# SuperScientificSoftwareLaboratory/DASP

Measured on AMD Instinct MI355X. Metric: SpMV GFLOP/s (f64), higher is better.
Workload: dtype f64; 1 GPU; HV15R synthetic stand-in (seeded; SuiteSparse dims/row statistics), A=1, x=1; rows=2017169, cols=2017169, nnz=275454726, partition=single GPU, generator_rev=26e32ff958e7, y_candidates=1

## Files before the change

dasp_amd/_lib.py:

```python
import ctypes as C
import os
import subprocess

_HERE = os.path.dirname(os.path.abspath(__file__))
SO_PATH = os.environ.get("DASP_AMD_SO") or os.path.join(_HERE, "libdasp_amd.so")


class DaspError(RuntimeError):
    def __init__(self, status, msg):
        super().__init__("dasp status %d: %s" % (status, msg))
        self.status = status


class Options(C.Structure):
    _fields_ = [
        ("threshold", C.c_double), ("block_longest", C.c_int), ("y_order", C.c_int), ("long_piece", C.c_int),
        ("host_threads", C.c_int), ("n_parts", C.c_int), ("part_bounds", C.POINTER(C.c_int)), ("part_stride", C.c_int),
        ("x_window", C.c_int), ("row_window", C.c_int), ("cid16", C.c_int), ("stream_policy", C.c_int),
        ("col_panels", C.c_int), ("slab_max_len", C.c_int), ("x_window_hybrid", C.c_int), ("piece_min_len", C.c_int),
        ("chunk_pairs", C.c_int), ("cid8", C.c_int), ("short_seg", C.c_int), ("row_tile_max", C.c_int), ("sort_columns", C.c_int),
        ("two_phase", C.c_int), ("tp_col_block", C.c_int), ("tp_row_block", C.c_int), ("long_cb", C.c_int),
        ("value_map", C.c_int),
    ]

# ... 109 lines not shown
    L.dasp_plan_panel.restype = vp
    L.dasp_plan_panel_range.argtypes = [vp, C.c_int, ip, ip]
    L.dasp_plan_upload.argtypes = [vp]
    L.dasp_plan_drop_host.argtypes = [vp]
    L.dasp_plan_update_values.argtypes = [vp, vp, vp]
    L.dasp_plan_update_values_host.argtypes = [vp, vp]
    L.dasp_plan_value_map_slots.argtypes = [vp]
    L.dasp_plan_value_map_slots.restype = C.c_longlong
    if hasattr(L, "dasp_plan_csr_fetch_bytes"):
        L.dasp_plan_csr_fetch_bytes.argtypes = [vp]
        L.dasp_plan_csr_fetch_bytes.restype = C.c_longlong
    if hasattr(L, "dasp_plan_shared_ids"):
        L.dasp_plan_shared_ids.argtypes = [vp, C.POINTER(C.c_longlong), C.POINTER(C.c_longlong), ip]
        L.dasp_plan_shared_ids_export.argtypes = [vp, C.c_char_p, vp, C.c_size_t]
        L.dasp_plan_shared_ids_export.restype = C.c_longlong
    L.dasp_plan_set_stream_policy.argtypes = [vp, C.c_int]
    if hasattr(L, "dasp_plan_set_tp_exact"):
        L.dasp_plan_set_tp_exact.argtypes = [vp, C.c_int]
        L.dasp_plan_tp_exact.argtypes = [vp]
        L.dasp_tp_exact_dot_f16.argtypes = [vp, vp, C.c_longlong, C.c_int, C.c_uint16, C.POINTER(C.c_uint16)]
    if hasattr(L, "dasp_plan_set_hub_exact"):
        L.dasp_plan_set_hub_exact.argtypes = [vp, C.c_int]
        L.dasp_plan_hub_exact.argtypes = [vp]
    if hasattr(L, "dasp_plan_set_f32_vectors"):
        fp = C.POINTER(C.c_float)
        L.dasp_plan_set_f32_vectors.argtypes = [vp, C.c_int]
        L.dasp_plan_f32_vectors.argtypes = [vp]
        L.dasp_plan_spmv_f32.argtypes = [vp, fp, fp, vp]
        L.dasp_plan_spmv_acc_f32.argtypes = [vp, fp, fp, vp]
    if hasattr(L, "dasp_plan_spmv_semiring_f32"):
# ... 46 lines not shown
    L.dasp_synth_generator.restype = C.c_char_p
    L.dasp_synth_row_lengths.argtypes = [C.c_char_p, C.c_double, C.c_int, C.c_int, vp]
    L.dasp_synth_rows.argtypes = [C.c_char_p, C.c_double, C.c_int, C.c_int, vp, vp]
    _lib = L
    return L


def check(rc):
    if rc != 0:
        raise DaspError(rc, lib().dasp_last_error().decode("utf-8", "replace"))


EXPORTS = (
    "dasp_last_error dasp_version dasp_mmio_allinone_f64 dasp_mmio_allinone_f16 dasp_free dasp_csr_save dasp_csr_load dasp_options_default "
    "dasp_plan_create dasp_plan_create_device dasp_plan_download_array dasp_plan_destroy dasp_plan_save dasp_plan_load dasp_plan_order dasp_plan_stats dasp_plan_y_order dasp_plan_x_len dasp_plan_panel_count dasp_plan_panel dasp_plan_panel_range dasp_plan_host_array dasp_plan_upload dasp_plan_tune_placement "
    "dasp_plan_drop_host dasp_plan_update_values dasp_plan_update_values_host dasp_plan_value_map_slots dasp_plan_csr_fetch_bytes dasp_plan_shared_ids dasp_plan_shared_ids_export dasp_plan_set_stream_policy dasp_plan_set_tp_exact dasp_plan_tp_exact dasp_plan_set_hub_exact dasp_plan_hub_exact dasp_tp_exact_dot_f16 dasp_plan_spmv dasp_plan_spmv_acc dasp_plan_set_f32_vectors dasp_plan_f32_vectors dasp_plan_spmv_f32 dasp_plan_spmv_acc_f32 dasp_plan_spmv_semiring_f32 dasp_plan_time dasp_plan_time_each dasp_plan_time_graph dasp_spmv_all_f64 dasp_spmv_all_f16 dasp_partition_rows "
    "dasp_selftest_mfma dasp_synth_dims dasp_synth_generator dasp_synth_row_lengths dasp_synth_rows "
    "dasp_mg_unique_id dasp_mg_plan_create dasp_mg_destroy dasp_mg_upload dasp_mg_comm_init dasp_mg_set_x dasp_mg_spmv dasp_mg_product dasp_mg_allgather "
    "dasp_mg_wait dasp_mg_get_y dasp_mg_get_y_local dasp_mg_y_local dasp_mg_gathered dasp_mg_x dasp_mg_subplan dasp_mg_info dasp_mg_check dasp_mg_set_fused dasp_mg_set_fake_exchange "
    "dasp_mg_push_export dasp_mg_push_connect dasp_mg_set_exchange dasp_mg_push_loopback dasp_mg_reserved_stream").split()
```

dasp_amd/api.py:

```python
import ctypes as C
import os

import numpy as np

from . import _lib
from ._lib import DaspError, Options, Stats

Y_PERMUTED, Y_NATURAL = 0, 1
MIN_PLUS, MIN_SECOND = 1, 2


def _vp(a):
    return a.ctypes.data_as(C.c_void_p)


def _dtype(precision):
    if precision == 64:
        return np.float64
    if precision == 16:
        return np.float16
    raise ValueError("precision must be 64 or 16")


def mmio_allinone(filename, precision=64):
# ... 212 lines not shown
        return {"available": bool(rc), "paired_id_bytes": int(pb.value), "shared_bytes": int(sb.value), "in_use": bool(use.value)}

    def shared_ids_export(self):
        out = []
        for what in (b"plane", b"table"):
            n = int(_lib.lib().dasp_plan_shared_ids_export(self._h, what, None, 0))
            if n < 0:
                _lib.check(n)
            a = np.empty(n // 4, np.uint32)
            n2 = int(_lib.lib().dasp_plan_shared_ids_export(self._h, what, a.ctypes.data_as(C.c_void_p), a.nbytes))
            if n2 < 0:
                _lib.check(n2)
            out.append(a)
        return out[0], out[1].reshape(-1, 4)

    @property
    def value_map_slots(self):
        n = int(_lib.lib().dasp_plan_value_map_slots(self._h))
        if n < 0:
            _lib.check(n)
        return n

    def kernel_variant(self):
        name = _lib.lib().dasp_debug_plan_kernel(self._h)
        if name is None:
            raise _lib.DaspError(-22, _lib.lib().dasp_last_error().decode("utf-8", "replace"))
        return name.decode()

    def set_stream_policy(self, policy):
        _lib.check(_lib.lib().dasp_plan_set_stream_policy(self._h, int(policy)))
# ... 139 lines not shown
```

dasp_amd/csrc/capi.cpp:

```cpp
#include <hip/hip_runtime_api.h>

#include <algorithm>
#include <cstdio>
#include <cstdlib>
#include <cstring>
#include <exception>
#include <memory>
#include <new>
#include <string>
#include <sys/stat.h>
#include <vector>

#include "plan.hpp"
#include "device.hpp"
#include "tp_exact.hpp"

namespace dasp {
const char *last_error_cstr();
int upload_plan(Plan &p);
int tune_placement(Plan &p, int trials, const void *dX, void *dY, double *ms_first, double *ms_kept);
int launch_spmv(Plan &p, const void *dX, void *dY, void *stream, bool accumulate);
int time_spmv_each(Plan &p, const void *dX, void *dY, void *stream, int warmup, int iters, float *ms_each);
int time_spmv(Plan &p, const void *dX, void *dY, void *stream, int warmup, int iters, double *wall_ms, double *event_ms);
int time_spmv_graph(Plan &p, const void *dX, void *dY, void *stream, int warmup, int iters, int batch, double *wall_ms, double *event_ms);
// ... 292 lines not shown
    return guarded("dasp_plan_shared_ids", [&] {
        long long pb = 0, sb = 0;
        if (!p.sh_known) {
            SharedIds sh;
            (void)derive_shared_ids(p, sh);
            p.sh_paired_bytes = sh.paired_id_bytes; p.sh_shared_bytes = sh.shared_bytes; p.sh_known = true;
        }
        pb = p.sh_paired_bytes; sb = p.sh_shared_bytes;
        if (pb == 0) return 0;
        if (paired_id_bytes) *paired_id_bytes = pb;
        if (shared_bytes) *shared_bytes = sb;
        return 1;
    });
}

long long dasp_plan_shared_ids_export(const dasp_plan_t *plan, const char *what, void *dst, size_t bytes)
{
    if (!plan || !what) return DASP_ERR_ARG;
    long long need = 0;
    const int rc = guarded("dasp_plan_shared_ids_export", [&] {
        const bool plane = std::strcmp(what, "plane") == 0;
        if (!plane && std::strcmp(what, "table") != 0) { set_error("dasp_plan_shared_ids_export: \"plane\" or \"table\""); return (int)DASP_ERR_ARG; }
        SharedIds sh;
        if (!derive_shared_ids(plan->impl, sh)) { set_error("the plan has no shared id plane (f64 with 16-bit ids, host arrays present, at least one pipelined block)"); return (int)DASP_ERR_STATE; }
        const std::vector<uint32_t> &v = plane ? sh.plane : sh.table;
        need = (long long)v.size() * 4;
        if (dst && bytes >= (size_t)need && need > 0) std::memcpy(dst, v.data(), (size_t)need);
        return (int)DASP_OK;
    });
    return rc != DASP_OK ? (long long)rc : need;
}

int dasp_plan_upload(dasp_plan_t *plan)
{
    if (!plan) return DASP_ERR_ARG;
// ... 254 lines not shown
```

dasp_amd/csrc/device.hpp:

```cpp
#pragma once

#include <cstddef>
#include <vector>

#include "plan.hpp"

namespace dasp {

struct ShortDev {
    int len, count, tiles, tile0;
    long long elem_off;
    SlotMap map;
    int seg, rpt;
};

struct DevArgs {
    const void *x;
    void *y;
    const void *long_val; const int *long_cid; const int *piece_ptr; const int *piece_dst; void *partial;
    const int *multi_ptr; const int *multi_dst;
    int n_pieces, n_multi;
    int pair_mode;
    const int *med_ptr; const void *med_val; const int *med_cid;
    const unsigned short *med_cid16; const int *med_base;
// ... 14 lines not shown
    int short_tpw, n_short_waves;
    int grp_wave0[kNumShortGroups];
    int grp_tile0[kNumShortGroups];
    const int *order;
    int wg_long, wg_med, wg_short;
    int xcd_on;
    int xcd_blk[9];
    int med_stride;
    const void *rt_val; const int *rt_cid; const int *rt_ptr; const unsigned short *rt_start; const unsigned long long *rt_mask;
    int n_rt_tiles, wg_rt, rt_max;
    const unsigned short *long_cid16; const int *long_base; const int *piece_c16;
    const int *med_nt;
    int wg_rot;
    int win_tiles;
    const unsigned char *med_shplane; const unsigned *med_shtab;
};

struct TpDev {
    const unsigned short *lcol; const int *dst; const int *unit;
    const void *val; const unsigned short *lrow; void *xs;
    const int *rb_row0; const int *rb_seg0;
    int n_units, n_rb, cb, rb_max, xlen, m;
};

struct LcbDev {
    const void *val; const unsigned short *lcol; const int *ptr; const int *unit; const int *row_dst; void *partial;
    int n_units, n_rows, n_cb, cb, xlen;
    void *xpart;
    int xsteps;
};
// ... 7 lines not shown
    void *dargs = nullptr;
    void *args_sent = nullptr;
    void *arena = nullptr;
    size_t arena_bytes = 0;
    ArenaMap map{};
    DevArgs args{};
    TpDev tp{};
    LcbDev lcb{};
    void *lcb_xpart = nullptr;
    void *wide_xs = nullptr, *wide_part = nullptr;
    bool nt = false;
    bool win1 = false;
    bool seven_waves = false;
    bool long16 = false;
    bool shared_ids = false;
    int device = -1;
    size_t ypart_stride = 0;
    void *vm_map = nullptr, *vm_runs = nullptr;
    bool vm_ready = false;
    void *pk_map[7] = {};
    int vm_n_runs = 0;
    long long vm_blocks = 0, vm_slots = 0;
    std::vector<Plan *> vm_arenas;
};
int value_map_upload(Plan &p);
void value_map_free(DevicePlan *d);


int require_device();
int upload_plan(Plan &p);
// ... 48 lines not shown
```

dasp_amd/csrc/mgstep.hip:

```cpp
#include <hip/hip_runtime.h>

#include <algorithm>
#include <cstdlib>
#include <string>
#include <vector>

#include "spmv_device.hpp"
#include "mgx_device.hpp"

namespace dasp {

struct StepCtl {
    const unsigned long long *gathered;
    unsigned long long need;
    const unsigned char *mark;
    const unsigned *mark_members;
    int n_marked, n_mark_shards;
    unsigned *mark_shards, *mark_top;
    unsigned long long *own_go;
    unsigned *all_shards, *all_top;
    unsigned long long *ready;
    unsigned long long step;
    int *err;
    int grid_a, grid_b, n_poll;
// ... 177 lines not shown
        hipError_t e_ = (expr);                                                                \
        if (e_ != hipSuccess) {                                                                \
            set_error(std::string(#expr) + ": " + hipGetErrorString(e_));                      \
            return e_ == hipErrorNoDevice ? DASP_ERR_NO_DEVICE : DASP_ERR_HIP;                 \
        }                                                                                      \
    } while (0)

int launch_mg_step(Plan &own, Plan *other, const void *x_own, const void *x_gathered, void *y, const MgStepCtl &h, void *stream)
{
    if (!mg_step_supported(own, other)) { set_error("plans do not qualify for the fused multi-GPU step"); return DASP_ERR_STATE; }
    DevArgs a = own.dev->args, b = other ? other->dev->args : own.dev->args;
    a.x = x_own; a.y = y; a.acc = 0;
    b.x = x_gathered; b.y = y; b.acc = 0;
    a.wg_med = (a.n_blocks + kWavesPerWG - 1) / kWavesPerWG; a.xcd_on = 0;
    b.wg_med = (b.n_blocks + kWavesPerWG - 1) / kWavesPerWG; b.xcd_on = 0;
    StepCtl c{};
    char *w = static_cast<char *>(h.words);
    c.mark_shards = reinterpret_cast<unsigned *>(w); c.all_shards = reinterpret_cast<unsigned *>(w + 8192);
    c.mark_top = reinterpret_cast<unsigned *>(w + 16384); c.all_top = reinterpret_cast<unsigned *>(w + 16384 + 256);
    c.gathered = reinterpret_cast<const unsigned long long *>(w + kMgWordGathered); c.need = other ? h.need : 0;
    c.own_go = reinterpret_cast<unsigned long long *>(w + kMgWordOwnGo);
    c.ready = reinterpret_cast<unsigned long long *>(w + kMgWordReady); c.step = h.step; c.err = h.err ? static_cast<int *>(h.err) : reinterpret_cast<int *>(w + kMgWordErr);
    c.grid_a = a.wg_long + a.wg_med + a.wg_short;
    c.grid_b = other ? b.wg_long + b.wg_med + b.wg_short : 0;
    c.n_poll = std::min(c.grid_b, std::max(1, h.max_pollers));
    c.poll_at = std::max(0, std::min(c.grid_a, (int)((double)c.grid_a * h.poll_at)));
    c.xcd_fenced = reinterpret_cast<unsigned long long *>(w + kMgWordXcd);
    c.mark = static_cast<const unsigned char *>(h.mark); c.mark_members = static_cast<const unsigned *>(h.mark_members);
    c.n_marked = other ? h.n_marked : 0; c.n_mark_shards = h.n_mark_shards;
    c.blk_order = static_cast<const int *>(h.blk_order);
// ... 29 lines not shown
}

int launch_mg_flag(void *word, unsigned long long value, void *stream)
{
    hipLaunchKernelGGL(dasp_mg_flag_kernel, dim3(1), dim3(64), 0, static_cast<hipStream_t>(stream), static_cast<unsigned long long *>(word), value);
    HIP_TRY(hipGetLastError());
    return DASP_OK;
}

int launch_mg_step2(Plan &plan, const void *x, void *y, const MgStep2Ctl &h, const MgPushArgs &push, void *stream)
{
    if (!mg_step_supported(plan, nullptr)) { set_error("plan does not qualify for the one-stream multi-GPU step"); return DASP_ERR_STATE; }
    DevArgs a = plan.dev->args;
    a.x = x; a.y = y; a.acc = 0;
    a.wg_med = (a.n_blocks + kWavesPerWG - 1) / kWavesPerWG; a.xcd_on = 0;
    Step2Ctl c{};
    c.wg_list = static_cast<const int *>(h.wg_list); c.blk_order = static_cast<const int *>(h.blk_order);
    c.n_push = h.n_push; c.n_free = h.n_free; c.n_marked = h.n_marked; c.n_total = h.n_total;
    c.n_poll = h.max_pollers > 0 ? std::max(1, std::min(h.n_marked, h.max_pollers)) : 0;
    c.arrived = static_cast<const unsigned long long *>(h.arrived); c.world = h.world; c.rank = h.rank; c.need = h.need;
    c.err = static_cast<int *>(h.err); c.timeout = h.timeout_ticks; c.sleep = std::max(1, h.poll_sleep);
    c.fence_mode = h.fence_mode; c.xcd_fenced = static_cast<unsigned long long *>(h.xcd_fenced); c.step = h.step;
    if (c.n_total != a.wg_long + a.wg_med + a.wg_short || c.n_free + c.n_marked > c.n_total) { set_error("one-stream step: the workgroup list does not match the plan's grid"); return DASP_ERR_STATE; }
    if (c.n_poll == 0 && c.n_marked == 0 && c.need) c.n_poll = 1;
    const int grid = c.n_push + (c.n_poll ? c.n_total - c.n_marked + c.n_poll : c.n_total);
    hipStream_t s = static_cast<hipStream_t>(stream);
    if (plan.dev->nt) hipLaunchKernelGGL((dasp_mg_step2_kernel<true>), dim3(grid), dim3(256), 0, s, a, push, c);
    else hipLaunchKernelGGL((dasp_mg_step2_kernel<false>), dim3(grid), dim3(256), 0, s, a, push, c);
    HIP_TRY(hipGetLastError());
    return DASP_OK;
// ... 4 lines not shown
```

dasp_amd/csrc/plan.hpp:

```cpp
#pragma once

#include <cstddef>
#include <cstdint>
#include <memory>
#include <string>
#include <utility>
#include <vector>

#include "../../include/dasp_amd.h"

namespace dasp {

template <class T>
struct NoInit : std::allocator<T> {
    template <class U> struct rebind { using other = NoInit<U>; };
    NoInit() = default;
    template <class U> NoInit(const NoInit<U> &) {}
    template <class U> void construct(U *p) noexcept { ::new (static_cast<void *>(p)) U; }
    template <class U, class... A> void construct(U *p, A &&...a) { ::new (static_cast<void *>(p)) U(std::forward<A>(a)...); }
};
template <class T> using raw_vector = std::vector<T, NoInit<T>>;

constexpr int kWave = 64;
constexpr long long kStreamBytes = 256ll << 20;
// ... 221 lines not shown
    TwoPhase tp;
    bool tp_exact = false;
    bool hub_exact = false;
    bool f32_vectors = false;

    bool value_map = false;
    std::vector<uint32_t> long_map, med_map, irr_map, short_map, rt_map;
    const uint32_t *map_src = nullptr;
    bool loaded = false;

    bool host_dropped = false;
    long long csr_fetch_bytes = 0;
    mutable long long sh_paired_bytes = 0, sh_shared_bytes = 0;
    mutable bool sh_known = false;
    bool sh_in_use = false;
    DevicePlan *dev = nullptr;

    ~Plan();
};

struct SharedIds {
    std::vector<uint32_t> plane, table;
    long long paired_id_bytes = 0;
    long long shared_bytes = 0;
    int n_pipelined = 0;
};
bool shared_ids_qualify(const Plan &p);
bool derive_shared_ids(const Plan &p, SharedIds &out);

struct DevCsr { const int *rp, *ci; const void *val; const uint32_t *src = nullptr; };
struct PackMeta {
    const std::vector<int> *ridL = nullptr; const std::vector<long long> *startL = nullptr;
    const raw_vector<int> *ridM = nullptr, *lenM = nullptr;
    const std::vector<int> *glist[kNumShortGroups] = {};
};
int devpack_validate(const Plan &p, const DevCsr &d);
int devpack_window_spans(const Plan &p, const DevCsr &d, const raw_vector<int> &ridW, int R, int *lo, int *hi, long long *wnnz);
int devpack_line_scatter(const Plan &p, const DevCsr &d, const std::vector<int> &rows, long long *lines, long long *entries);
int devpack_row_coherence(const Plan &p, const DevCsr &d, const std::vector<int> &rows, int within, long long *near, long long *entries);
int devpack_chunk_spans(const Plan &p, const DevCsr &d, const raw_vector<int> &ridM, const raw_vector<int> &lenM,
                        const std::vector<int> &nchunks, int *k16, unsigned long long *narrow_mask);
int devpack_densest_spans(const Plan &p, const DevCsr &d, const raw_vector<int> &ridW, const raw_vector<int> &lenW, int R, const std::vector<int> &wlist,
                          long long cap_cols, int A, int *hmin, long long *hin);
// ... 72 lines not shown
```

dasp_amd/csrc/sharedids.cpp:

```cpp
#include <cstring>

#include "plan.hpp"

namespace dasp {

bool shared_ids_qualify(const Plan &p)
{
    if (p.precision != 64 || !p.cid16 || p.windowed || p.two_phase || !p.panels.empty() || p.panel || p.host_dropped) return false;
    const size_t nb = p.med_ptr.empty() ? 0 : p.med_ptr.size() - 1;
    if (nb == 0 || p.med_c8ptr.size() != nb + 1 || p.irr_ptr.size() < 2) return false;
    return p.med_cid8.size() == p.cnt_reg8 && p.med_cid16.size() == p.cnt_reg - p.cnt_reg8 && p.cnt_reg > 0;
}

bool derive_shared_ids(const Plan &p, SharedIds &out)
{
    out = SharedIds();
    if (!shared_ids_qualify(p)) return false;
    constexpr int CH = 64, K = 4;
    const size_t nb = p.med_ptr.size() - 1;
    out.table.assign(4 * nb, 0u);
    const unsigned char *c8 = p.med_cid8.data();
    const unsigned char *c16 = reinterpret_cast<const unsigned char *>(p.med_cid16.data());
    std::vector<const unsigned char *> slot;
    for (size_t b = 0; b < nb; ++b) {
// ... 27 lines not shown
        uint32_t *dst = out.plane.data() + at;
        for (const unsigned char *s : slot)
            for (int kq = 0; kq < 4; ++kq)
                for (int g = 0; g < L; ++g) std::memcpy(dst++, s + 4 * (rep[g] + 16 * kq), 4);
        out.table[4 * b] = (uint32_t)ranks; out.table[4 * b + 1] = (uint32_t)(ranks >> 32);
        out.table[4 * b + 2] = (uint32_t)(at / 4); out.table[4 * b + 3] = (uint32_t)L;
        out.paired_id_bytes += (long long)slot.size() * 4 * CH;
        ++out.n_pipelined;
        if (at / 4 > 0xFFFFFFFFull) { out = SharedIds(); return false; }
    }
    if (out.n_pipelined == 0) { out = SharedIds(); return false; }
    out.shared_bytes = (long long)out.plane.size() * 4 + (long long)out.table.size() * 4;
    return true;
}

}
```

dasp_amd/csrc/spmv_device.hpp:

```cpp
#pragma once
#include <hip/hip_runtime.h>

#include <cstdint>

#include "plan.hpp"
#include "device.hpp"

namespace dasp {

typedef double f64x4 __attribute__((ext_vector_type(4)));
typedef double f64x2 __attribute__((ext_vector_type(2)));
typedef float f32x4 __attribute__((ext_vector_type(4)));
typedef _Float16 f16x4 __attribute__((ext_vector_type(4)));
typedef int i32x4 __attribute__((ext_vector_type(4)));
typedef int i32x2 __attribute__((ext_vector_type(2)));
typedef unsigned short u16x4 __attribute__((ext_vector_type(4)));
typedef unsigned short u16x8 __attribute__((ext_vector_type(8)));
typedef const __attribute__((address_space(1))) unsigned char *gbyte_p;
typedef _Float16 f16x8 __attribute__((ext_vector_type(8)));


template <bool NT, class U>
__device__ __forceinline__ U ldg(const U *p)
{
// ... 56 lines not shown
template <class U> __device__ __forceinline__ U *ldp(U *const *field)
{
    typedef __attribute__((address_space(1))) U *gptr;
    return (U *)*reinterpret_cast<const __attribute__((address_space(4))) gptr *>(reinterpret_cast<uintptr_t>(field));
}
__device__ __forceinline__ DevArgs load_args(const CallArgs &c)
{
    static_assert(sizeof(DevArgs) % 4 == 0, "DevArgs is a whole number of words");
    int w[sizeof(DevArgs) / 4];
#pragma unroll
    for (int i = 0; i < (int)(sizeof(DevArgs) / 4); ++i) w[i] = tab<true>(reinterpret_cast<const int *>(c.plan), i);
    DevArgs a;
    __builtin_memcpy(&a, w, sizeof a);
#define DASP_G(f) a.f = ldp(&c.plan->f)
    DASP_G(long_val); DASP_G(long_cid); DASP_G(long_cid16); DASP_G(long_base); DASP_G(piece_c16); DASP_G(piece_ptr); DASP_G(piece_dst); DASP_G(partial); DASP_G(multi_ptr); DASP_G(multi_dst);
    DASP_G(med_ptr); DASP_G(med_val); DASP_G(med_cid); DASP_G(med_cid16); DASP_G(med_base); DASP_G(med_cid8); DASP_G(med_c8ptr); DASP_G(med_shplane); DASP_G(med_shtab);
    DASP_G(irr_ptr); DASP_G(med_nt); DASP_G(irr_val); DASP_G(irr_cid); DASP_G(med_dst); DASP_G(win_cmin); DASP_G(win_len);
    DASP_G(short_val); DASP_G(short_cid); DASP_G(groups); DASP_G(order);
    DASP_G(rt_val); DASP_G(rt_cid); DASP_G(rt_ptr); DASP_G(rt_start); DASP_G(rt_mask);
#undef DASP_G
    a.x = c.x; a.y = c.y; a.acc = c.acc; a.ywt = c.ywt;
    return a;
}

template <int I, int N> struct LastLE {
    static __device__ __forceinline__ void run(const int (&arr)[N], int w, int &idx, int &val)
    {
        if constexpr (I < N) { const bool in = w >= arr[I]; idx = in ? I : idx; val = in ? arr[I] : val; LastLE<I + 1, N>::run(arr, w, idx, val); }
    }
};
template <int I, int N> struct PickPair {
// ... 501 lines not shown
                for (int j = 0; j < 4; ++j) { f.a[j] = ok ? f.a[j] : (_Float16)0; f.b[j] = ok ? f.b[j] : (_Float16)0; }
            }
            frag_mfma(acc, f);
        }
    }
    part_t d;
    const bool on_diag = diag_of(acc, lane, d);
    const part_t total = wave_sum(on_diag ? d : (part_t)0);
    if (lane == 0) {
        const int dst = tab<true>(a.piece_dst, p);
        if (dst >= 0) put_y<T, YS>(a, dst, total);
        else static_cast<part_t *>(a.partial)[~dst] = total;
    }
}

template <class T, int L, bool NT, int YS = 0>
__device__ __forceinline__ void short_rows(const DevArgs &a, const ShortDev &g, int local_tile, int lane)
{
    constexpr int SR = Tr<T>::SHORT_ROWS;
    constexpr int V = SR / kWave;
    const T *x = static_cast<const T *>(a.x);
    const T *val = static_cast<const T *>(a.short_val);
    using part_t = typename Tr<T>::part_t;
    part_t s[V];
#pragma unroll
    for (int v = 0; v < V; ++v) s[v] = 0;
    const size_t base = (size_t)g.elem_off + (size_t)local_tile * L * SR + (size_t)V * lane;
#pragma unroll
    for (int k = 0; k < L; ++k) {
        if constexpr (V == 2) {
// ... 243 lines not shown
#ifndef DASP_WIN64_U
#define DASP_WIN64_U 3
#define DASP_WIN64_S 6
#endif
template <class T, bool NT, bool C16, bool WIN, bool C8, bool RT = false, bool W64 = false, bool L16 = false, bool SH = false>
__device__ __forceinline__ void spmv_body(const DevArgs &a, char *lds_raw, int wg_index, Stamps &st)
{
    const int lane = threadIdx.x & 63;
    const int wave = __builtin_amdgcn_readfirstlane(threadIdx.x >> 6);
    int wg = wg_index;
    if constexpr (sizeof(T) == 2 && !WIN && !RT) {
        if (a.wg_rot) { const int grid = a.wg_long + a.wg_med + a.wg_short; wg += a.wg_rot; wg = wg >= grid ? wg - grid : wg; }
    }
    const int wpw = WIN ? a.wpw : kWavesPerWG;
    if (wg < a.wg_long) {
        const int p = wg * wpw + wave;
        if (p < a.n_pieces) long_piece<T, NT, 0, !WIN, L16 && !WIN>(a, p, lane);
    } else if (wg < a.wg_long + a.wg_med) {
        st.kind = 1;
        if constexpr (!WIN) {
            const int m = wg - a.wg_long;
            const XGlobal<T> x{static_cast<const T *>(a.x)};
            if (a.xcd_on) {
                const int k = m & 7;
                int lo = a.xcd_blk[0], hi = a.xcd_blk[1];
                PickPair<1, 9>::run(a.xcd_blk, k, lo, hi);
                const int b = lo + (m >> 3) * kWavesPerWG + wave;
                if (b < hi) medium_block<T, NT, C16, 0, C8, 0, false, 0, 0, SH>(a, b, lane, x);
            } else if (sizeof(T) == 8 && !a.med_stride) {
                const int b = m * kWavesPerWG + wave;
                if (b < a.n_blocks) medium_block<T, NT, C16, 0, C8, 0, false, 0, 0, SH>(a, b, lane, x);
// ... 113 lines not shown
```

dasp_amd/csrc/upload.cpp:

```cpp
#include <hip/hip_runtime_api.h>

#include <algorithm>
#include <chrono>
#include <cmath>
#include <cstdio>
#include <cstdlib>
#include <cstring>
#include <string>
#include <type_traits>
#include <vector>

#include "plan.hpp"
#include "device.hpp"

namespace dasp {

#define HIP_TRY(expr)                                                                          \
    do {                                                                                       \
        hipError_t e_ = (expr);                                                                \
        if (e_ != hipSuccess) {                                                                \
            set_error(std::string(#expr) + ": " + hipGetErrorString(e_));                      \
            return e_ == hipErrorNoDevice ? DASP_ERR_NO_DEVICE : DASP_ERR_HIP;                 \
        }                                                                                      \
    } while (0)
// ... 82 lines not shown
    }
    if (narrow_elems) *narrow_elems = narrow;
    return on;
}
void choose_long16(Plan &p)
{
    DevicePlan *d = p.dev;
    if (!d) return;
    d->long16 = long16_rule(p, nullptr);
}

long long shared_ids_net_saving(const Plan &p, const SharedIds &s, bool long16)
{
    long long narrow = 0;
    (void)long16_rule(p, &narrow);
    return s.paired_id_bytes - s.shared_bytes - (long16 ? 2 * narrow : 0);
}
static bool seven_waves_rule(const Plan &p)
{
    bool on = false;
    if (p.precision == 64 && !p.windowed && p.med_ptr.size() > 1 && p.irr_ptr.size() > 1) {
        long long one = 0, all = 0;
        const int K = p.geo.med_k, nbk = (int)p.med_ptr.size() - 1;
        for (int b = 0; b < nbk; ++b) {
            const int nc = p.med_ptr[(size_t)b + 1] - p.med_ptr[(size_t)b], r0 = b * kMedRows;
            const int nt = (p.irr_ptr[(size_t)r0 + 1] - p.irr_ptr[(size_t)r0] + K - 1) / K;
            all += nc + nt;
            if (med_oneshot64(nc, nt)) one += nc + nt;
        }
        on = all > 0 && one * 10 >= all * 7 && p.stats.data_X > (64ll << 20);
        if (const char *e = std::getenv("DASP_SEVEN_WAVES")) on = std::atoi(e) != 0;
// ... 169 lines not shown
    const size_t o_mdst = add(p.med_dst.data(), p.med_dst.size() * 4);
    const size_t o_wc = add(p.win_cmin.data(), p.win_cmin.size() * 4);
    const size_t o_wl = add(p.win_len.data(), p.win_len.size() * 4);
    const size_t o_sv = add(src_of(p.short_val), p.cnt_short * vbytes);
    const size_t o_sc = add(src_of(p.short_cid), p.cnt_short * 4);
    const size_t o_g = add(groups.data(), groups.size() * sizeof(ShortDev));
    const size_t o_rv = add(src_of(p.rt_val), p.cnt_rt * vbytes);
    const size_t o_rc = add(src_of(p.rt_cid), p.cnt_rt * 4);
    const size_t o_rp = add(p.rt_ptr.data(), p.rt_ptr.size() * 4);
    const size_t o_rs = add(p.rt_start.data(), p.rt_start.size() * 2);
    const size_t o_rm = add(p.rt_mask.data(), p.rt_mask.size() * 8);
    std::vector<int> ord_mapped;
    if (natural && !p.dst_map.empty()) { ord_mapped.resize(p.order.size()); for (size_t i = 0; i < p.order.size(); ++i) ord_mapped[i] = p.dst_map[(size_t)p.order[i]]; }
    const size_t o_ord = add(natural ? (ord_mapped.empty() ? p.order.data() : ord_mapped.data()) : nullptr, natural ? p.order.size() * 4 : 0);
    SharedIds sh;
    size_t o_shp = 0, o_sht = 0;
    d->shared_ids = false;
    p.sh_in_use = false;
    if (share_ids_env() != 0 && (p.stats.data_X > kStreamBytes || share_ids_env() == 1)) {
        const bool have = derive_shared_ids(p, sh);
        p.sh_paired_bytes = sh.paired_id_bytes; p.sh_shared_bytes = sh.shared_bytes; p.sh_known = true;
        p.sh_in_use = d->shared_ids = have && shared_ids_rule(p, sh);
        if (d->shared_ids) { o_shp = add(sh.plane.data(), sh.plane.size() * 4); o_sht = add(sh.table.data(), sh.table.size() * 4); }
    }

    HIP_TRY(hipMalloc(&d->arena, total));
    d->arena_bytes = total;
    if (std::getenv("DASP_VERBOSE")) std::fprintf(stderr, "[dasp upload] arena %p + %zu bytes\n", d->arena, total);
    char *base = static_cast<char *>(d->arena);
    for (const Item &it : items)
        if (it.src && it.bytes) HIP_TRY(hipMemcpy(base + it.off, it.src, it.bytes, hipMemcpyHostToDevice));

    d->map.long_val = o_lv; d->map.long_cid = o_lc; d->map.med_val = o_mv; d->map.med_cid = o_mc; d->map.med_cid16 = o_mc16; d->map.med_cid8 = o_mc8;
    d->map.med_base = o_mb; d->map.irr_val = o_iv; d->map.irr_cid = o_ic; d->map.short_val = o_sv; d->map.short_cid = o_sc;
    d->map.rt_val = o_rv; d->map.rt_cid = o_rc; d->map.long_cid16 = o_lc16; d->map.long_base = o_lb; d->map.piece_c16 = o_pc16;
    DevArgs &a = d->args;
    a.long_val = base + o_lv; a.long_cid = (const int *)(base + o_lc);
    a.long_cid16 = (const unsigned short *)(base + o_lc16); a.long_base = (const int *)(base + o_lb); a.piece_c16 = (const int *)(base + o_pc16);
    a.piece_ptr = (const int *)(base + o_pp); a.piece_dst = (const int *)(base + o_pd);
    a.multi_ptr = (const int *)(base + o_mp); a.multi_dst = (const int *)(base + o_md);
    a.partial = base + o_part;
    a.n_pieces = (int)p.piece_dst.size(); a.n_multi = (int)p.multi_dst.size();
    a.med_ptr = (const int *)(base + o_mptr); a.med_val = base + o_mv; a.med_cid = (const int *)(base + o_mc);
    a.irr_ptr = (const int *)(base + o_ip); a.med_nt = (const int *)(base + o_mnt); a.irr_val = base + o_iv; a.irr_cid = (const int *)(base + o_ic);
    a.n_blocks = p.stats.n_med_blocks; a.row_block = p.n_mfma_rows; a.row_long = p.med_slot0;
    for (int g = 0; g < kNumShortGroups; ++g) a.grp_tile0[g] = p.grp[g].tile0;
    a.short_val = base + o_sv; a.short_cid = (const int *)(base + o_sc); a.groups = (const ShortDev *)(base + o_g);
    a.n_short_tiles = p.stats.n_short_tiles;
    a.order = natural ? (const int *)(base + o_ord) : nullptr;
    a.wpw = p.windowed ? std::min(16, p.row_window / kMedRows) : kWavesPerWG;
    a.wg_long = (a.n_pieces + a.wpw - 1) / a.wpw;
    a.med_cid16 = (const unsigned short *)(base + o_mc16); a.med_base = (const int *)(base + o_mb);
    a.med_cid8 = (const unsigned char *)(base + o_mc8); a.med_c8ptr = (const int *)(base + o_c8p);
    a.med_shplane = d->shared_ids ? (const unsigned char *)(base + o_shp) : nullptr; a.med_shtab = d->shared_ids ? (const unsigned *)(base + o_sht) : nullptr;
    a.med_dst = (const int *)(base + o_mdst); a.win_cmin = (const int *)(base + o_wc); a.win_len = (const int *)(base + o_wl);
    a.n_windows = (int)p.win_len.size(); a.blocks_per_win = p.windowed ? p.row_window / kMedRows : 0;
    a.win_hybrid = p.win_hybrid ? 1 : 0; a.win_rel16 = p.win_rel16 ? 1 : 0; a.pair_mode = p.pair_mode;
    a.win_xcd = 1;
    a.skip0 = p.panel ? 1 : 0;
    if (const char *e = std::getenv("DASP_WIN_XCD")) a.win_xcd = std::atoi(e);
    d->win1 = false;
    d->seven_waves = false;
    choose_long16(p);
    d->seven_waves = seven_waves_rule(p);
    if (p.windowed) {
        int cus = 256;
// ... 67 lines not shown
    }
    return sync_dev_args(p);
}


static void rebase_args(DevArgs &a, const char *from, const char *to, size_t bytes)
{
    auto mv = [&](auto &ptr) {
        const char *q = reinterpret_cast<const char *>(ptr);
        if (q >= from && q < from + bytes) ptr = reinterpret_cast<std::remove_reference_t<decltype(ptr)>>(const_cast<char *>(to + (q - from)));
    };
    mv(a.long_val); mv(a.long_cid); mv(a.long_cid16); mv(a.long_base); mv(a.piece_c16); mv(a.piece_ptr); mv(a.piece_dst); mv(a.partial); mv(a.multi_ptr); mv(a.multi_dst);
    mv(a.med_ptr); mv(a.med_val); mv(a.med_cid); mv(a.med_cid16); mv(a.med_base); mv(a.med_cid8); mv(a.med_c8ptr);
    mv(a.irr_ptr); mv(a.med_nt); mv(a.irr_val); mv(a.irr_cid); mv(a.med_dst); mv(a.win_cmin); mv(a.win_len);
    mv(a.short_val); mv(a.short_cid); mv(a.groups); mv(a.order);
    mv(a.med_shplane); mv(a.med_shtab);
}

int tune_placement(Plan &p, int trials, const void *dX, void *dY, double *ms_first, double *ms_kept)
{
    DevicePlan *d = p.dev;
    if (ms_first) *ms_first = 0.0;
    if (ms_kept) *ms_kept = 0.0;
    if (trials <= 0) trials = 2;
    trials = std::min(trials, 8);
    if (!d || !d->arena || trials <= 1 || d->arena_bytes < (size_t(256) << 20) || !p.panels.empty() || p.panel || p.windowed || p.two_phase) return DASP_OK;
    const bool verbose = std::getenv("DASP_VERBOSE") != nullptr;
    const size_t vb = (size_t)p.geo.vbytes, bytes = d->arena_bytes;
    const size_t xlen = p.opt.n_parts > 0 ? (size_t)p.opt.n_parts * (size_t)p.opt.part_stride : (size_t)p.n;
    void *x = nullptr, *y = nullptr;
    const void *ux = dX; void *uy = dY;
// ... 70 lines not shown
```

include/dasp_amd.h:

```cpp
#ifndef DASP_AMD_H
#define DASP_AMD_H

#include <stddef.h>
#include <stdint.h>

#ifdef __cplusplus
extern "C" {
#endif

typedef enum dasp_status {
    DASP_OK = 0,
    DASP_ERR_OPEN = -1,
    DASP_ERR_BANNER = -2,
    DASP_ERR_SIZE = -4,
    DASP_ERR_ENTRY = -5,
    DASP_ERR_ARG = -10,
    DASP_ERR_NOMEM = -11,
    DASP_ERR_NO_DEVICE = -20,
    DASP_ERR_HIP = -21,
    DASP_ERR_STATE = -22
} dasp_status;

const char *dasp_last_error(void);
const char *dasp_version(void);
// ... 103 lines not shown
dasp_plan_t *dasp_plan_panel(dasp_plan_t *plan, int k);
int dasp_plan_panel_range(const dasp_plan_t *plan, int k, int *col_begin, int *col_end);

long long dasp_plan_host_array(const dasp_plan_t *plan, const char *name, const void **ptr, int *elem_bytes);

int dasp_plan_upload(dasp_plan_t *plan);
int dasp_plan_drop_host(dasp_plan_t *plan);

int dasp_plan_update_values(dasp_plan_t *plan, const void *dVal, void *stream);
int dasp_plan_update_values_host(dasp_plan_t *plan, const void *csrVal);
long long dasp_plan_value_map_slots(const dasp_plan_t *plan);
long long dasp_plan_csr_fetch_bytes(const dasp_plan_t *plan);

int dasp_plan_shared_ids(const dasp_plan_t *plan, long long *paired_id_bytes, long long *shared_bytes, int *in_use);
long long dasp_plan_shared_ids_export(const dasp_plan_t *plan, const char *what, void *dst, size_t bytes);

int dasp_plan_set_stream_policy(dasp_plan_t *plan, int policy);

int dasp_plan_set_tp_exact(dasp_plan_t *plan, int on);
int dasp_plan_tp_exact(const dasp_plan_t *plan);
int dasp_plan_set_hub_exact(dasp_plan_t *plan, int on);
int dasp_plan_hub_exact(const dasp_plan_t *plan);
int dasp_tp_exact_dot_f16(const uint16_t *a, const uint16_t *x, long long n, int accumulate, uint16_t y_in, uint16_t *y_out);

int dasp_plan_spmv(dasp_plan_t *plan, const void *dX, void *dY, void *stream);
int dasp_plan_spmv_acc(dasp_plan_t *plan, const void *dX, void *dY, void *stream);

int dasp_plan_set_f32_vectors(dasp_plan_t *plan, int on);
int dasp_plan_f32_vectors(const dasp_plan_t *plan);
int dasp_plan_spmv_f32(dasp_plan_t *plan, const float *dX, float *dY, void *stream);
// ... 79 lines not shown
```

Baseline: 1285 GFLOP/s.

## Share column-id lists across consecutive long pieces with identical sparsity

Adds a long-unit table that groups up to eight consecutive long pieces whose column-id lists are identical. A wave then loads the ids and gathers x once and reuses them across the group, streaming only the values for each piece. This cuts index traffic and repeated x gathers in the long-row stage. In exchange it adds a table lookup per wave, gives less parallelism per group, and applies only when the shared-id path is enabled and such twin pieces exist.

New measurement: 1320 GFLOP/s, median of 6. 1.03x the previous value.

```diff
diff --git a/dasp_amd/_lib.py b/dasp_amd/_lib.py
--- a/dasp_amd/_lib.py
+++ b/dasp_amd/_lib.py
@@ -147,6 +147,8 @@
         L.dasp_plan_shared_ids.argtypes = [vp, C.POINTER(C.c_longlong), C.POINTER(C.c_longlong), ip]
         L.dasp_plan_shared_ids_export.argtypes = [vp, C.c_char_p, vp, C.c_size_t]
         L.dasp_plan_shared_ids_export.restype = C.c_longlong
+    if hasattr(L, "dasp_plan_shared_long_ids"):
+        L.dasp_plan_shared_long_ids.argtypes = [vp, C.POINTER(C.c_longlong), ip]
     L.dasp_plan_set_stream_policy.argtypes = [vp, C.c_int]
     if hasattr(L, "dasp_plan_set_tp_exact"):
         L.dasp_plan_set_tp_exact.argtypes = [vp, C.c_int]
@@ -223,7 +225,7 @@
 EXPORTS = (
     "dasp_last_error dasp_version dasp_mmio_allinone_f64 dasp_mmio_allinone_f16 dasp_free dasp_csr_save dasp_csr_load dasp_options_default "
     "dasp_plan_create dasp_plan_create_device dasp_plan_download_array dasp_plan_destroy dasp_plan_save dasp_plan_load dasp_plan_order dasp_plan_stats dasp_plan_y_order dasp_plan_x_len dasp_plan_panel_count dasp_plan_panel dasp_plan_panel_range dasp_plan_host_array dasp_plan_upload dasp_plan_tune_placement "
-    "dasp_plan_drop_host dasp_plan_update_values dasp_plan_update_values_host dasp_plan_value_map_slots dasp_plan_csr_fetch_bytes dasp_plan_shared_ids dasp_plan_shared_ids_export dasp_plan_set_stream_policy dasp_plan_set_tp_exact dasp_plan_tp_exact dasp_plan_set_hub_exact dasp_plan_hub_exact dasp_tp_exact_dot_f16 dasp_plan_spmv dasp_plan_spmv_acc dasp_plan_set_f32_vectors dasp_plan_f32_vectors dasp_plan_spmv_f32 dasp_plan_spmv_acc_f32 dasp_plan_spmv_semiring_f32 dasp_plan_time dasp_plan_time_each dasp_plan_time_graph dasp_spmv_all_f64 dasp_spmv_all_f16 dasp_partition_rows "
+    "dasp_plan_drop_host dasp_plan_update_values dasp_plan_update_values_host dasp_plan_value_map_slots dasp_plan_csr_fetch_bytes dasp_plan_shared_ids dasp_plan_shared_ids_export dasp_plan_shared_long_ids dasp_plan_set_stream_policy dasp_plan_set_tp_exact dasp_plan_tp_exact dasp_plan_set_hub_exact dasp_plan_hub_exact dasp_tp_exact_dot_f16 dasp_plan_spmv dasp_plan_spmv_acc dasp_plan_set_f32_vectors dasp_plan_f32_vectors dasp_plan_spmv_f32 dasp_plan_spmv_acc_f32 dasp_plan_spmv_semiring_f32 dasp_plan_time dasp_plan_time_each dasp_plan_time_graph dasp_spmv_all_f64 dasp_spmv_all_f16 dasp_partition_rows "
     "dasp_selftest_mfma dasp_synth_dims dasp_synth_generator dasp_synth_row_lengths dasp_synth_rows "
     "dasp_mg_unique_id dasp_mg_plan_create dasp_mg_destroy dasp_mg_upload dasp_mg_comm_init dasp_mg_set_x dasp_mg_spmv dasp_mg_product dasp_mg_allgather "
     "dasp_mg_wait dasp_mg_get_y dasp_mg_get_y_local dasp_mg_y_local dasp_mg_gathered dasp_mg_x dasp_mg_subplan dasp_mg_info dasp_mg_check dasp_mg_set_fused dasp_mg_set_fake_exchange "
diff --git a/dasp_amd/api.py b/dasp_amd/api.py
--- a/dasp_amd/api.py
+++ b/dasp_amd/api.py
@@ -250,6 +250,27 @@
             out.append(a)
         return out[0], out[1].reshape(-1, 4)
 
+    def shared_long_ids(self):
+        fig, use = (C.c_longlong * 5)(), C.c_int(0)
+        rc = _lib.lib().dasp_plan_shared_long_ids(self._h, fig, C.byref(use))
+        if rc < 0:
+            _lib.check(rc)
+        return {"available": bool(rc), "long_id_bytes": int(fig[0]), "grouped_id_bytes": int(fig[1]), "units": int(fig[2]), "groups": int(fig[3]),
+                "rows_in_groups": int(fig[4]), "in_use": bool(use.value)}
+
+    def shared_long_ids_export(self):
+        out = []
+        for what in (b"long_units", b"long_plane"):
+            n = int(_lib.lib().dasp_plan_shared_ids_export(self._h, what, None, 0))
+            if n < 0:
+                _lib.check(n)
+            a = np.empty(n // 4, np.uint32)
+            n2 = int(_lib.lib().dasp_plan_shared_ids_export(self._h, what, a.ctypes.data_as(C.c_void_p), a.nbytes))
+            if n2 < 0:
+                _lib.check(n2)
+            out.append(a)
+        return out[0].reshape(-1, 4), out[1].view(np.int32)
+
     @property
     def value_map_slots(self):
         n = int(_lib.lib().dasp_plan_value_map_slots(self._h))
diff --git a/dasp_amd/csrc/capi.cpp b/dasp_amd/csrc/capi.cpp
--- a/dasp_amd/csrc/capi.cpp
+++ b/dasp_amd/csrc/capi.cpp
@@ -330,11 +330,39 @@
     });
 }
 
+int dasp_plan_shared_long_ids(const dasp_plan_t *plan, long long fig[5], int *in_use)
+{
+    if (!plan) return DASP_ERR_ARG;
+    const Plan &p = plan->impl;
+    if (fig) for (int i = 0; i < 5; ++i) fig[i] = 0;
+    if (in_use) *in_use = p.dev && p.shl_in_use ? 1 : 0;
+    return guarded("dasp_plan_shared_long_ids", [&] {
+        long long f[5] = {0, 0, 0, 0, 0};
+        if (p.dev && p.shl_known) for (int i = 0; i < 5; ++i) f[i] = p.shl_fig[i];
+        else {
+            SharedIds sh;
+            if (derive_long_units(p, sh)) { f[0] = sh.long_id_bytes; f[1] = sh.long_shared_bytes; f[2] = sh.n_long_units(); f[3] = sh.n_long_groups; f[4] = sh.n_long_grouped; }
+        }
+        if (f[2] == 0) return 0;
+        if (fig) for (int i = 0; i < 5; ++i) fig[i] = f[i];
+        return 1;
+    });
+}
+
 long long dasp_plan_shared_ids_export(const dasp_plan_t *plan, const char *what, void *dst, size_t bytes)
 {
     if (!plan || !what) return DASP_ERR_ARG;
     long long need = 0;
     const int rc = guarded("dasp_plan_shared_ids_export", [&] {
+        if (std::strcmp(what, "long_units") == 0 || std::strcmp(what, "long_plane") == 0) {
+            SharedIds sh;
+            if (!derive_long_units(plan->impl, sh)) { set_error("the plan has no long unit table (f64 with 16-bit ids, host arrays present, at least one long piece)"); return (int)DASP_ERR_STATE; }
+            const bool units = std::strcmp(what, "long_units") == 0;
+            const void *src = units ? (const void *)sh.long_units.data() : (const void *)sh.long_plane.data();
+            need = (long long)(units ? sh.long_units.size() : sh.long_plane.size()) * 4;
+            if (dst && bytes >= (size_t)need && need > 0) std::memcpy(dst, src, (size_t)need);
+            return (int)DASP_OK;
+        }
         const bool plane = std::strcmp(what, "plane") == 0;
         if (!plane && std::strcmp(what, "table") != 0) { set_error("dasp_plan_shared_ids_export: \"plane\" or \"table\""); return (int)DASP_ERR_ARG; }
         SharedIds sh;
diff --git a/dasp_amd/csrc/device.hpp b/dasp_amd/csrc/device.hpp
--- a/dasp_amd/csrc/device.hpp
+++ b/dasp_amd/csrc/device.hpp
@@ -52,6 +52,8 @@
     int wg_rot;
     int win_tiles;
     const unsigned char *med_shplane; const unsigned *med_shtab;
+    const unsigned *long_units; const int *long_shplane;
+    int n_long_units, long_pad_;
 };
 
 struct TpDev {
@@ -89,6 +91,7 @@
     bool seven_waves = false;
     bool long16 = false;
     bool shared_ids = false;
+    bool shared_long = false;
     int device = -1;
     size_t ypart_stride = 0;
     void *vm_map = nullptr, *vm_runs = nullptr;
diff --git a/dasp_amd/csrc/mgstep.hip b/dasp_amd/csrc/mgstep.hip
--- a/dasp_amd/csrc/mgstep.hip
+++ b/dasp_amd/csrc/mgstep.hip
@@ -215,6 +215,7 @@
     b.x = x_gathered; b.y = y; b.acc = 0;
     a.wg_med = (a.n_blocks + kWavesPerWG - 1) / kWavesPerWG; a.xcd_on = 0;
     b.wg_med = (b.n_blocks + kWavesPerWG - 1) / kWavesPerWG; b.xcd_on = 0;
+    a.wg_long = (a.n_pieces + kWavesPerWG - 1) / kWavesPerWG; b.wg_long = (b.n_pieces + kWavesPerWG - 1) / kWavesPerWG;
     StepCtl c{};
     char *w = static_cast<char *>(h.words);
     c.mark_shards = reinterpret_cast<unsigned *>(w); c.all_shards = reinterpret_cast<unsigned *>(w + 8192);
@@ -274,6 +275,7 @@
     DevArgs a = plan.dev->args;
     a.x = x; a.y = y; a.acc = 0;
     a.wg_med = (a.n_blocks + kWavesPerWG - 1) / kWavesPerWG; a.xcd_on = 0;
+    a.wg_long = (a.n_pieces + kWavesPerWG - 1) / kWavesPerWG;
     Step2Ctl c{};
     c.wg_list = static_cast<const int *>(h.wg_list); c.blk_order = static_cast<const int *>(h.blk_order);
     c.n_push = h.n_push; c.n_free = h.n_free; c.n_marked = h.n_marked; c.n_total = h.n_total;
diff --git a/dasp_amd/csrc/plan.hpp b/dasp_amd/csrc/plan.hpp
--- a/dasp_amd/csrc/plan.hpp
+++ b/dasp_amd/csrc/plan.hpp
@@ -259,6 +259,9 @@
     mutable long long sh_paired_bytes = 0, sh_shared_bytes = 0;
     mutable bool sh_known = false;
     bool sh_in_use = false;
+    mutable long long shl_fig[5] = {0, 0, 0, 0, 0};
+    mutable bool shl_known = false;
+    bool shl_in_use = false;
     DevicePlan *dev = nullptr;
 
     ~Plan();
@@ -269,9 +272,17 @@
     long long paired_id_bytes = 0;
     long long shared_bytes = 0;
     int n_pipelined = 0;
-};
+    std::vector<uint32_t> long_units;
+    std::vector<int32_t> long_plane;
+    long long long_id_bytes = 0;
+    long long long_shared_bytes = 0;
+    int n_long_groups = 0, n_long_grouped = 0;
+    int n_long_units() const { return (int)(long_units.size() / 4); }
+};
+constexpr int kLongGroupMax = 8;
 bool shared_ids_qualify(const Plan &p);
 bool derive_shared_ids(const Plan &p, SharedIds &out);
+bool derive_long_units(const Plan &p, SharedIds &out);
 
 struct DevCsr { const int *rp, *ci; const void *val; const uint32_t *src = nullptr; };
 struct PackMeta {
diff --git a/dasp_amd/csrc/sharedids.cpp b/dasp_amd/csrc/sharedids.cpp
--- a/dasp_amd/csrc/sharedids.cpp
+++ b/dasp_amd/csrc/sharedids.cpp
@@ -1,3 +1,4 @@
+#include <cstdlib>
 #include <cstring>
 
 #include "plan.hpp"
@@ -65,4 +66,41 @@
     return true;
 }
 
+bool derive_long_units(const Plan &p, SharedIds &out)
+{
+    out.long_units.clear(); out.long_plane.clear();
+    out.long_id_bytes = out.long_shared_bytes = 0;
+    out.n_long_groups = out.n_long_grouped = 0;
+    if (!shared_ids_qualify(p)) return false;
+    const size_t P = p.piece_dst.size();
+    if (P == 0 || p.piece_ptr.size() != P + 1 || p.long_cid.size() != p.cnt_long || (size_t)p.piece_ptr[P] > p.long_cid.size()) return false;
+    constexpr int CH = 64;
+    const char *env = std::getenv("DASP_SHARE_LONG");
+    const bool off = env && std::atoi(env) == 0;
+    const int *cid = p.long_cid.data();
+    long long single_elems = 0;
+    out.long_units.reserve(4 * P);
+    for (size_t q = 0; q < P;) {
+        const int e0 = p.piece_ptr[q], len = p.piece_ptr[q + 1] - e0;
+        size_t g = 1;
+        if (!off && p.piece_dst[q] >= 0 && len > 0 && len <= kMedShot64 * CH)
+            while (g < (size_t)kLongGroupMax && q + g < P && p.piece_dst[q + g] >= 0 && p.piece_ptr[q + g + 1] - p.piece_ptr[q + g] == len &&
+                   std::memcmp(cid + e0, cid + p.piece_ptr[q + g], (size_t)len * 4) == 0) ++g;
+        uint32_t at = 0;
+        if (g >= 2) {
+            if (out.long_plane.size() > 0xFFFFFFFFull - 1024) { out.long_units.clear(); out.long_plane.clear(); out.n_long_groups = out.n_long_grouped = 0; return false; }
+            at = (uint32_t)out.long_plane.size();
+            out.long_plane.insert(out.long_plane.end(), cid + e0, cid + e0 + len);
+            out.long_plane.resize((out.long_plane.size() + 3) & ~size_t(3), -1);
+            ++out.n_long_groups; out.n_long_grouped += (int)g;
+        } else single_elems += len;
+        const uint32_t e[4] = {(uint32_t)q, (uint32_t)g, at, 0u};
+        out.long_units.insert(out.long_units.end(), e, e + 4);
+        q += g;
+    }
+    out.long_id_bytes = 4ll * p.piece_ptr[P];
+    out.long_shared_bytes = 4 * single_elems + 4ll * (long long)out.long_plane.size() + 4ll * (long long)out.long_units.size();
+    return true;
 }
+
+}
diff --git a/dasp_amd/csrc/spmv_device.hpp b/dasp_amd/csrc/spmv_device.hpp
--- a/dasp_amd/csrc/spmv_device.hpp
+++ b/dasp_amd/csrc/spmv_device.hpp
@@ -94,7 +94,7 @@
     __builtin_memcpy(&a, w, sizeof a);
 #define DASP_G(f) a.f = ldp(&c.plan->f)
     DASP_G(long_val); DASP_G(long_cid); DASP_G(long_cid16); DASP_G(long_base); DASP_G(piece_c16); DASP_G(piece_ptr); DASP_G(piece_dst); DASP_G(partial); DASP_G(multi_ptr); DASP_G(multi_dst);
-    DASP_G(med_ptr); DASP_G(med_val); DASP_G(med_cid); DASP_G(med_cid16); DASP_G(med_base); DASP_G(med_cid8); DASP_G(med_c8ptr); DASP_G(med_shplane); DASP_G(med_shtab);
+    DASP_G(med_ptr); DASP_G(med_val); DASP_G(med_cid); DASP_G(med_cid16); DASP_G(med_base); DASP_G(med_cid8); DASP_G(med_c8ptr); DASP_G(med_shplane); DASP_G(med_shtab); DASP_G(long_units); DASP_G(long_shplane);
     DASP_G(irr_ptr); DASP_G(med_nt); DASP_G(irr_val); DASP_G(irr_cid); DASP_G(med_dst); DASP_G(win_cmin); DASP_G(win_len);
     DASP_G(short_val); DASP_G(short_cid); DASP_G(groups); DASP_G(order);
     DASP_G(rt_val); DASP_G(rt_cid); DASP_G(rt_ptr); DASP_G(rt_start); DASP_G(rt_mask);
@@ -626,6 +626,69 @@
     }
 }
 
+template <bool NT, int N>
+__device__ __forceinline__ void long_group_steps(const DevArgs &a, int p, int G, int p0, int len, const int *ids, int lane)
+{
+    constexpr int CH = Tr<double>::CHUNK;
+    const double *x = static_cast<const double *>(a.x);
+    const int tail = len - (N - 1) * CH;
+    const bool ok = lane < tail;
+    const int last = ok ? (N - 1) * CH + lane : 0;
+    int c[N];
+#pragma unroll
+    for (int i = 0; i + 1 < N; ++i) c[i] = ldg<NT>(ids + i * CH + lane);
+    c[N - 1] = ldg<NT>(ids + last);
+    const double *v = static_cast<const double *>(a.long_val) + p0;
+    double cur[N];
+#pragma unroll
+    for (int i = 0; i + 1 < N; ++i) cur[i] = ldg<NT>(v + i * CH + lane);
+    cur[N - 1] = ldg<NT>(v + last);
+    c[N - 1] = ok ? c[N - 1] : -1;
+    double b[N];
+#pragma unroll
+    for (int i = 0; i < N; ++i) { const double g = x[c[i] < 0 ? 0 : c[i]]; b[i] = c[i] < 0 ? 0.0 : g; }
+#pragma unroll 1
+    for (int t = 0; t < G; ++t) {
+        double nxt[N];
+        if (t + 1 < G) {
+            v += len;
+#pragma unroll
+            for (int i = 0; i + 1 < N; ++i) nxt[i] = ldg<NT>(v + i * CH + lane);
+            nxt[N - 1] = ldg<NT>(v + last);
+        } else {
+#pragma unroll
+            for (int i = 0; i < N; ++i) nxt[i] = 0.0;
+        }
+        f64x4 acc = {0, 0, 0, 0};
+        cur[N - 1] = ok ? cur[N - 1] : 0.0;
+#pragma unroll
+        for (int i = 0; i < N; ++i) acc = __builtin_amdgcn_mfma_f64_16x16x4f64(cur[i], b[i], acc, 0, 0, 0);
+        double d;
+        const bool on_diag = diag_of(acc, lane, d);
+        const double total = wave_sum(on_diag ? d : 0.0);
+        if (lane == 0) put_y<double, 0>(a, tab<true>(a.piece_dst, p + t), total);
+#pragma unroll
+        for (int i = 0; i < N; ++i) cur[i] = nxt[i];
+    }
+}
+template <bool NT, int N> struct LongGroupDispatch {
+    static __device__ __forceinline__ void run(const DevArgs &a, int p, int G, int p0, int len, int n, const int *ids, int lane)
+    {
+        if (n == N) long_group_steps<NT, N>(a, p, G, p0, len, ids, lane);
+        else LongGroupDispatch<NT, N - 1>::run(a, p, G, p0, len, n, ids, lane);
+    }
+};
+template <bool NT> struct LongGroupDispatch<NT, 0> {
+    static __device__ __forceinline__ void run(const DevArgs &, int, int, int, int, int, const int *, int) {}
+};
+template <bool NT>
+__device__ __forceinline__ void long_group(const DevArgs &a, int p, int G, unsigned at, int lane)
+{
+    constexpr int CH = Tr<double>::CHUNK;
+    const int p0 = tab<true>(a.piece_ptr, p), len = tab<true>(a.piece_ptr, p + 1) - p0;
+    LongGroupDispatch<NT, Tr<double>::LONG_SHOT>::run(a, p, G, p0, len, (len + CH - 1) / CH, a.long_shplane + at, lane);
+}
+
 template <class T, int L, bool NT, int YS = 0>
 __device__ __forceinline__ void short_rows(const DevArgs &a, const ShortDev &g, int local_tile, int lane)
 {
@@ -899,7 +962,23 @@
     }
     const int wpw = WIN ? a.wpw : kWavesPerWG;
     if (wg < a.wg_long) {
-        const int p = wg * wpw + wave;
+        int p = wg * wpw + wave;
+        if constexpr (SH) {
+            int G = 1; unsigned at = 0;
+            bool have = p < a.n_pieces;
+            if (a.long_units) {
+                have = p < a.n_long_units;
+                if (have) {
+                    typedef unsigned u32x4 __attribute__((ext_vector_type(4)));
+                    const u32x4 e = tab<true>(reinterpret_cast<const u32x4 *>(a.long_units), p);
+                    p = (int)e[0]; G = (int)e[1]; at = e[2];
+                }
+            }
+            if (!have) return;
+            if (G >= 2) long_group<NT>(a, p, G, at, lane);
+            else long_piece<T, NT, 0, !WIN, L16 && !WIN>(a, p, lane);
+            return;
+        }
         if (p < a.n_pieces) long_piece<T, NT, 0, !WIN, L16 && !WIN>(a, p, lane);
     } else if (wg < a.wg_long + a.wg_med) {
         st.kind = 1;
diff --git a/dasp_amd/csrc/upload.cpp b/dasp_amd/csrc/upload.cpp
--- a/dasp_amd/csrc/upload.cpp
+++ b/dasp_amd/csrc/upload.cpp
@@ -120,7 +120,8 @@
 {
     long long narrow = 0;
     (void)long16_rule(p, &narrow);
-    return s.paired_id_bytes - s.shared_bytes - (long16 ? 2 * narrow : 0);
+    const long long twins = s.n_long_groups > 0 ? s.long_id_bytes - s.long_shared_bytes : 0;
+    return s.paired_id_bytes - s.shared_bytes - (long16 ? 2 * narrow : 0) + twins;
 }
 static bool seven_waves_rule(const Plan &p)
 {
@@ -320,14 +321,19 @@
     if (natural && !p.dst_map.empty()) { ord_mapped.resize(p.order.size()); for (size_t i = 0; i < p.order.size(); ++i) ord_mapped[i] = p.dst_map[(size_t)p.order[i]]; }
     const size_t o_ord = add(natural ? (ord_mapped.empty() ? p.order.data() : ord_mapped.data()) : nullptr, natural ? p.order.size() * 4 : 0);
     SharedIds sh;
-    size_t o_shp = 0, o_sht = 0;
-    d->shared_ids = false;
-    p.sh_in_use = false;
+    size_t o_shp = 0, o_sht = 0, o_lgp = 0, o_lgu = 0;
+    d->shared_ids = d->shared_long = false;
+    p.sh_in_use = p.shl_in_use = p.shl_known = false;
     if (share_ids_env() != 0 && (p.stats.data_X > kStreamBytes || share_ids_env() == 1)) {
         const bool have = derive_shared_ids(p, sh);
         p.sh_paired_bytes = sh.paired_id_bytes; p.sh_shared_bytes = sh.shared_bytes; p.sh_known = true;
+        (void)derive_long_units(p, sh);
+        p.shl_fig[0] = sh.long_id_bytes; p.shl_fig[1] = sh.long_shared_bytes; p.shl_fig[2] = sh.n_long_units(); p.shl_fig[3] = sh.n_long_groups; p.shl_fig[4] = sh.n_long_grouped;
+        p.shl_known = true;
         p.sh_in_use = d->shared_ids = have && shared_ids_rule(p, sh);
         if (d->shared_ids) { o_shp = add(sh.plane.data(), sh.plane.size() * 4); o_sht = add(sh.table.data(), sh.table.size() * 4); }
+        p.shl_in_use = d->shared_long = d->shared_ids && sh.n_long_groups > 0;
+        if (d->shared_long) { o_lgp = add(sh.long_plane.data(), sh.long_plane.size() * 4); o_lgu = add(sh.long_units.data(), sh.long_units.size() * 4); }
     }
 
     HIP_TRY(hipMalloc(&d->arena, total));
@@ -355,7 +361,9 @@
     a.n_short_tiles = p.stats.n_short_tiles;
     a.order = natural ? (const int *)(base + o_ord) : nullptr;
     a.wpw = p.windowed ? std::min(16, p.row_window / kMedRows) : kWavesPerWG;
-    a.wg_long = (a.n_pieces + a.wpw - 1) / a.wpw;
+    a.long_units = d->shared_long ? (const unsigned *)(base + o_lgu) : nullptr; a.long_shplane = d->shared_long ? (const int *)(base + o_lgp) : nullptr;
+    a.n_long_units = d->shared_long ? sh.n_long_units() : 0; a.long_pad_ = 0;
+    a.wg_long = ((d->shared_long ? a.n_long_units : a.n_pieces) + a.wpw - 1) / a.wpw;
     a.med_cid16 = (const unsigned short *)(base + o_mc16); a.med_base = (const int *)(base + o_mb);
     a.med_cid8 = (const unsigned char *)(base + o_mc8); a.med_c8ptr = (const int *)(base + o_c8p);
     a.med_shplane = d->shared_ids ? (const unsigned char *)(base + o_shp) : nullptr; a.med_shtab = d->shared_ids ? (const unsigned *)(base + o_sht) : nullptr;
@@ -453,7 +461,7 @@
     mv(a.med_ptr); mv(a.med_val); mv(a.med_cid); mv(a.med_cid16); mv(a.med_base); mv(a.med_cid8); mv(a.med_c8ptr);
     mv(a.irr_ptr); mv(a.med_nt); mv(a.irr_val); mv(a.irr_cid); mv(a.med_dst); mv(a.win_cmin); mv(a.win_len);
     mv(a.short_val); mv(a.short_cid); mv(a.groups); mv(a.order);
-    mv(a.med_shplane); mv(a.med_shtab);
+    mv(a.med_shplane); mv(a.med_shtab); mv(a.long_units); mv(a.long_shplane);
 }
 
 int tune_placement(Plan &p, int trials, const void *dX, void *dY, double *ms_first, double *ms_kept)
diff --git a/include/dasp_amd.h b/include/dasp_amd.h
--- a/include/dasp_amd.h
+++ b/include/dasp_amd.h
@@ -141,6 +141,7 @@
 
 int dasp_plan_shared_ids(const dasp_plan_t *plan, long long *paired_id_bytes, long long *shared_bytes, int *in_use);
 long long dasp_plan_shared_ids_export(const dasp_plan_t *plan, const char *what, void *dst, size_t bytes);
+int dasp_plan_shared_long_ids(const dasp_plan_t *plan, long long fig[5], int *in_use);
 
 int dasp_plan_set_stream_policy(dasp_plan_t *plan, int policy);
 
```
